# saifahmadgit/go2-sim2real-locomotion-rl

Hardware: AMD Instinct MI355X
Metric: env-steps/sec (all envs) Go2 walk 4096 envs; 1/2/4/8-GPU scaling (higher is better)
Workload: dtype f32

## Files before the change

### go2_sim2real_locomotion_rl_amd/build.py

```python
import os
import shutil
import subprocess
import sys

_HERE = os.path.dirname(os.path.abspath(__file__))
REPO_ROOT = os.path.dirname(_HERE)
HIP_SRC = os.path.join(_HERE, "csrc", "go2sim.hip")
HIP_SRC_POLICY = os.path.join(_HERE, "csrc", "go2sim_policy.hip")
HIP_HDR_GJK = os.path.join(_HERE, "csrc", "go2sim_gjk_dev.h")
HIP_LIB = os.path.join(_HERE, "csrc", "libgo2sim.so")
ORACLE_SRC = os.path.join(REPO_ROOT, "oracle", "go2sim_cpu.cpp")
ORACLE_SRC_POLICY = os.path.join(REPO_ROOT, "oracle", "policy_cpu.cpp")
ORACLE_LIB = os.path.join(REPO_ROOT, "oracle", "libgo2sim_cpu.so")
ORACLE_LIB_FAST = os.path.join(REPO_ROOT, "oracle", "libgo2sim_cpu_fast.so")

HIP_FLAGS = ["--offload-arch=gfx950", "-O3", "-std=c++17", "-ffp-contract=off", "-fPIC", "-shared", "-Wall", "-Wno-unused-function",
             "-Wno-unused-const-variable"]
CPU_FLAGS = ["-O2", "-std=c++17", "-ffp-contract=off", "-fopenmp", "-fPIC", "-shared", "-Wall", "-Wno-unused-function", "-Wno-unused-variable"]


def _newer(target, *sources):
    if not os.path.exists(target):
        return False
    t = os.path.getmtime(target)
# ... 36 lines not shown
        cmd = ["g++", *CPU_FLAGS, *extra, ORACLE_SRC, ORACLE_SRC_POLICY, "-o", lib]
        if verbose:
            print("[build]", " ".join(cmd), file=sys.stderr)
        subprocess.run(cmd, check=True)
    return ORACLE_LIB


def build_oracle_variant(name, extra_flags, force=False, verbose=True):
    out = os.path.join(REPO_ROOT, "oracle", f"libgo2sim_cpu_{name}.so")
    deps = [ORACLE_SRC, ORACLE_SRC_POLICY, os.path.join(REPO_ROOT, "oracle", "gjk_epa_cpu.h"), *_headers()]
    if not force and _newer(out, *deps):
        return out
    cmd = ["g++", *CPU_FLAGS, *extra_flags, ORACLE_SRC, ORACLE_SRC_POLICY, "-o", out]
    if verbose:
        print("[build]", " ".join(cmd), file=sys.stderr)
    subprocess.run(cmd, check=True)
    return out


HIP_VARIANTS = {
    "bracket_inline": ["-DGO2SIM_BRACKET_INLINE"],
    "rng_const": ["-DGO2SIM_RNG_CONST"],
    "strict": ["-DGO2SIM_FAST_ORDER=0"],
}
ORACLE_VARIANTS = {
    "rng_const": ["-DGO2SIM_RNG_CONST"],
    "rng_const_fast": ["-DGO2SIM_RNG_CONST", "-DGO2SIM_FAST_ORDER"],
}


SHAPES = {
    "pendulum": dict(NL=3, ND=1, NQ=1, NG=2, NJ=1),
    "double_pendulum": dict(NL=4, ND=2, NQ=2, NG=3, NJ=2),
    "box": dict(NL=2, ND=6, NQ=7, NG=2, NJ=1),
}


def _shape_flags(name):
    return [f"-DGO2SIM_{k}={v}" for k, v in SHAPES[name].items()]


def build_shape_variant(name, hip=True, force=False, verbose=True):
    cpu = build_oracle_variant("shape_" + name, _shape_flags(name), force=force, verbose=verbose)
    gpu = build_hip_variant("shape_" + name, ["-DGO2SIM_FAST_ORDER=0", *_shape_flags(name)], force=force, verbose=verbose) if hip else None
    return cpu, gpu

# ... 22 lines not shown
```

### go2_sim2real_locomotion_rl_amd/csrc/go2sim.hip

```cpp

#include <hip/hip_runtime.h>

#include <cstdint>
#include <cstdio>
#include <cstdlib>
#include <cstring>
#include <new>
#include <vector>

#include "../../include/go2sim.h"
#include "../../include/go2sim_detmath.h"

#define DEV __device__ __forceinline__
#define DEVN __device__ __noinline__

namespace {

constexpr int NL = GO2SIM_NL, ND = GO2SIM_ND, NQ = GO2SIM_NQ, NG = GO2SIM_NG, NJ = GO2SIM_NJ;
constexpr int NPAIR = GO2SIM_NPAIR_MAX, MAXC = GO2SIM_MAX_CONTACTS, MAXB = GO2SIM_MAX_BROAD, MAXR = GO2SIM_MAX_ROWS;
constexpr int JOINT_FIXED = 0, JOINT_REVOLUTE = 1, JOINT_FREE = 4;
constexpr int GEOM_PLANE = 0, GEOM_SPHERE = 1, GEOM_CYLINDER = 3, GEOM_BOX = 5, GEOM_TERRAIN = 7;
constexpr int TERRAIN_CB = 4;
constexpr int MAX_CONTACTS_PER_PAIR = 5;
constexpr int CTRL_FORCE = 0, CTRL_VELOCITY = 1, CTRL_POSITION = 2;
// ... 168 lines not shown
  ovel = cross(s_ang, m_vel) + cross(s_vel, m_ang);
  oang = cross(s_ang, m_ang);
}
DEV void orthogonals(V3 a, V3& b, V3& c) {
  if (dm_abs(a.y) < 0.5f) b = v3(-a.x * a.y, 1.0f - a.y * a.y, -a.z * a.y);
  else b = v3(-a.x * a.z, -a.y * a.z, 1.0f - a.z * a.z);
  b = normalized(b);
  c = cross(a, b);
}
DEV void imp_aref(const float* p, float neg_penetration, float vel, float pos, float& imp, float& aref) {
  float timeconst = p[0], dampratio = p[1], dmin = p[2], dmax = p[3], width = p[4], mid = p[5], power = p[6];
  float imp_x = dm_abs(neg_penetration) / width;
  float imp_a = (1.0f / dm_pow(mid, power - 1.0f)) * dm_pow(imp_x, power);
  float imp_b = 1.0f - (1.0f / dm_pow(1.0f - mid, power - 1.0f)) * dm_pow(1.0f - imp_x, power);
  float imp_y = (imp_x < mid) ? imp_a : imp_b;
  imp = dmin + imp_y * (dmax - dmin);
  imp = clampf(imp, dmin, dmax);
  imp = (imp_x > 1.0f) ? dmax : imp;
  float b = 2.0f / (dmax * timeconst);
  float k = 1.0f / (dmax * dmax * timeconst * timeconst * dampratio * dampratio);
  aref = -b * vel - k * imp * pos;
}

struct Link {
  int parent, root, entity, is_fixed, joint_start, joint_end, dof_start, dof_end, q_start, q_end, n_dofs, geom_start, geom_end;
  V3 pos; Q4 quat; V3 inertial_pos; Q4 inertial_quat; M3 inertial_i; float mass; float invweight[2];
};
struct Joint { int type, link, q_start, dof_start, dof_end; V3 pos; float sol_params[7]; };
struct Dof { V3 motion_ang, motion_vel; float limit[2], invweight, armature, damping, stiffness, frictionloss, kp, kv, force_range[2]; };
struct Geom { int type, link, is_convex; V3 pos; Q4 quat; float data[7], friction, sol_params[7]; V3 center; V3 aabb[8]; float rim[32][2]; };
struct Entity { int link_start, link_end, dof_start, dof_end, geom_start, geom_end; };
struct Model {
  int n_links, n_joints, n_dofs, n_qs, n_geoms, n_entities, n_pairs, max_collision_pairs, max_contact_pairs, max_broad_pairs,
      n_contacts_per_pair, iterations, ls_iterations, ccd_iterations, support_res;
  float substep_dt; V3 gravity; float eps, tolerance, ls_tolerance, meaninertia, mc_perturbation, mc_tolerance, mpr_to_gjk_ratio, ccd_eps,
      ccd_tolerance;
  Link links[NL]; Joint joints[NJ]; Dof dofs[ND]; Geom geoms[NG]; Entity entities[2];
  float qpos0[NQ]; float mass_parent_mask[ND][ND]; int pair_idx[NG][NG]; int theta_to_ring[180];
  int pair_list[NPAIR];
  int terrain_enabled, terrain_rows, terrain_cols; float terrain_hs; float terrain_xyz_maxmin[6]; const float* terrain_hf;
  const float* terrain_cmax; int terrain_crows, terrain_ccols;
  int n_levels, level_start[NL + 1], level_links[NL], child_start[NL + 1], child_list[NL], dof_link[ND];
  int arrow_mode;
};

bool parse_model(const void* blob, size_t nbytes, Model& m) {
  m.terrain_enabled = 0; m.terrain_rows = m.terrain_cols = 0; m.terrain_hs = 0.0f; m.terrain_hf = nullptr;
  m.terrain_cmax = nullptr; m.terrain_crows = m.terrain_ccols = 0;
  if (nbytes < 128) return false;
  const int32_t* H = (const int32_t*)blob;
  if (H[0] != GO2SIM_MODEL_MAGIC || H[1] != GO2SIM_MODEL_VERSION) return false;
  m.n_links = H[2]; m.n_joints = H[3]; m.n_dofs = H[4]; m.n_qs = H[5]; m.n_geoms = H[6]; m.n_entities = H[7];
  m.n_pairs = H[8]; m.max_collision_pairs = H[9]; m.max_contact_pairs = H[10]; m.max_broad_pairs = H[11];
  m.n_contacts_per_pair = H[12]; m.iterations = H[13]; m.ls_iterations = H[14]; m.ccd_iterations = H[15]; m.support_res = H[16];
  int nf = H[18], ni = H[19];
  if (m.n_links != NL || m.n_joints != NJ || m.n_dofs != ND || m.n_qs != NQ || m.n_geoms != NG || m.n_entities != 2) return false;
  if (m.n_pairs > NPAIR || m.max_contact_pairs > MAXC || m.max_broad_pairs > MAXB || m.support_res != 180 || H[17] != 32) return false;
  if (m.n_contacts_per_pair > MAX_CONTACTS_PER_PAIR) return false;
  if (nbytes < 128 + (size_t)4 * (nf + ni)) return false;
  const float* F = (const float*)((const char*)blob + 128);
  const int32_t* I = (const int32_t*)(F + nf);
  const float* f = F;
  m.substep_dt = f[0]; m.gravity = {f[1], f[2], f[3]}; m.eps = f[4]; m.tolerance = f[5]; m.ls_tolerance = f[6]; m.meaninertia = f[7];
  m.mc_perturbation = f[8]; m.mc_tolerance = f[9]; m.mpr_to_gjk_ratio = f[10]; m.ccd_eps = f[11]; m.ccd_tolerance = f[12];
  f += 16;
  for (int i = 0; i < NL; ++i, f += 26) {
// ... 61 lines not shown
    for (int i = 0; i < NL; ++i) {
      int par = m.links[i].parent;
      if (par >= i) return false;
      depth[i] = (par < 0) ? 0 : depth[par] + 1;
      if (depth[i] > max_depth) max_depth = depth[i];
    }
    m.n_levels = max_depth + 1;
    int k = 0;
    for (int lev = 0; lev <= max_depth; ++lev) {
      m.level_start[lev] = k;
      for (int i = 0; i < NL; ++i) if (depth[i] == lev) m.level_links[k++] = i;
    }
    for (int lev = max_depth + 1; lev <= NL; ++lev) m.level_start[lev] = k;
    k = 0;
    for (int par = 0; par < NL; ++par) {
      m.child_start[par] = k;
      for (int i = NL - 1; i > par; --i) if (m.links[i].parent == par) m.child_list[k++] = i;
    }
    m.child_start[NL] = k;
    for (int d = 0; d < ND; ++d) m.dof_link[d] = -1;
    for (int i = 0; i < NL; ++i) for (int d = m.links[i].dof_start; d < m.links[i].dof_end; ++d) m.dof_link[d] = i;
    for (int d = 0; d < ND; ++d) if (m.dof_link[d] < 0) return false;
  }
  int g_next = 0;
  for (int i = 0; i < NL; ++i) { if (m.links[i].geom_start != g_next) return false; g_next = m.links[i].geom_end; }
  return g_next == NG;
}


struct LinkS {
  int parent, entity, is_fixed, joint_start, joint_end, dof_start, dof_end, q_start, q_end, n_dofs;
  V3 pos; Q4 quat; V3 inertial_pos; Q4 inertial_quat; M3 inertial_i; float mass; float invweight[2];
};
struct GeomS { int type, link; V3 pos; Q4 quat; };
struct JLim { int q_start, dof_start; float lo, hi; };
constexpr int NTRI = ND * (ND + 1) / 2;
constexpr int LEG_K = 4, LEG_D = 3;
struct alignas(16) ModelS {
  int n_levels, iterations, ls_iterations, arrow_mode;
  float substep_dt; V3 gravity; float eps, tolerance, ls_tolerance, meaninertia;
  LinkS links[NL];
  unsigned char tri_i[NTRI + 1], tri_j[NTRI + 1];
  JLim jlim[NJ];
  Joint joints[NJ]; Dof dofs[ND]; GeomS geoms[NG]; Entity entities[2];
  float qpos0[NQ]; unsigned mass_mask_bits[ND];
  int level_start[NL + 1], level_links[NL], child_start[NL + 1], child_list[NL], dof_link[ND];
// ... 62 lines not shown
      float v = m.mass_parent_mask[i][j];
      if (v == 1.0f) bits |= 1u << j; else if (v != 0.0f) return false;
    }
    o.mass_mask_bits[i] = bits;
  }
  for (int i = 0; i <= NL; ++i) { o.level_start[i] = m.level_start[i]; o.child_start[i] = m.child_start[i]; }
  for (int i = 0; i < NL; ++i) { o.level_links[i] = m.level_links[i]; o.child_list[i] = m.child_list[i]; }
  for (int i = 0; i < ND; ++i) o.dof_link[i] = m.dof_link[i];
  int k = 0;
  for (int i = 0; i < ND; ++i) for (int j = 0; j <= i; ++j) { o.tri_i[k] = (unsigned char)i; o.tri_j[k] = (unsigned char)j; k++; }
  for (int i = 0; i < NJ; ++i) {
    const Joint& J = m.joints[i];
    bool rev = J.type == JOINT_REVOLUTE;
    o.jlim[i].q_start = rev ? J.q_start : -1; o.jlim[i].dof_start = J.dof_start;
    o.jlim[i].lo = rev ? m.dofs[J.dof_start].limit[0] : 0.0f; o.jlim[i].hi = rev ? m.dofs[J.dof_start].limit[1] : 0.0f;
  }
  o.leg_form = build_leg_form(m, o) ? 1 : 0;
  return true;
}
DEV float mass_mask(const ModelS& m, int i, int j) { return (float)((m.mass_mask_bits[i] >> j) & 1u); }
DEV void tri_index(const ModelS& m, int idx, int& i, int& j) { i = m.tri_i[idx]; j = m.tri_j[idx]; }

struct ModelView {
  int n_levels, iterations, ls_iterations, arrow_mode, leg_form; float substep_dt; V3 gravity; float eps, tolerance, ls_tolerance, meaninertia;
  const LinkS* links; const Joint* joints; const Dof* dofs; const GeomS* geoms; const Entity* entities; const float* qpos0;
  const unsigned* mass_mask_bits; const int *level_start, *level_links, *child_start, *child_list, *dof_link; const unsigned char *tri_i, *tri_j;
  const unsigned char* leg_links; int leg_root;
  DEV ModelView(const ModelS* t, const ModelS* __restrict__ g)
      : n_levels(g->n_levels), iterations(g->iterations), ls_iterations(g->ls_iterations), arrow_mode(g->arrow_mode), leg_form(g->leg_form), substep_dt(g->substep_dt), gravity(g->gravity), eps(g->eps),
        tolerance(g->tolerance), ls_tolerance(g->ls_tolerance), meaninertia(g->meaninertia), links(t->links), joints(t->joints), dofs(t->dofs),
        geoms(t->geoms), entities(t->entities), qpos0(t->qpos0), mass_mask_bits(t->mass_mask_bits), level_start(t->level_start),
        level_links(t->level_links), child_start(t->child_start), child_list(t->child_list), dof_link(t->dof_link), tri_i(t->tri_i), tri_j(t->tri_j),
        leg_links(t->leg_links), leg_root(g->leg_root) {}
  DEV ModelView(const LinkS* lds_links, const unsigned char* lds_tri_i, const unsigned char* lds_tri_j, const Model* __restrict__ g)
      : n_levels(g->n_levels), iterations(g->iterations), ls_iterations(g->ls_iterations), arrow_mode(g->arrow_mode), leg_form(0), substep_dt(g->substep_dt), gravity(g->gravity), eps(g->eps),
        tolerance(g->tolerance), ls_tolerance(g->ls_tolerance), meaninertia(g->meaninertia), links(lds_links), joints(g->joints), dofs(g->dofs),
        geoms(nullptr), entities(g->entities), qpos0(g->qpos0), mass_mask_bits(nullptr), level_start(nullptr), level_links(nullptr), child_start(nullptr),
        child_list(nullptr), dof_link(nullptr), tri_i(lds_tri_i), tri_j(lds_tri_j), leg_links(nullptr), leg_root(-1) {}
};
DEV float mass_mask(const ModelView& m, int i, int j) { return (float)((m.mass_mask_bits[i] >> j) & 1u); }
DEV void tri_index(const ModelView& m, int idx, int& i, int& j) { i = m.tri_i[idx]; j = m.tri_j[idx]; }
constexpr int lds_dma_bytes(int nbytes) { return (nbytes + 1023) / 1024 * 1024; }
template <int NBYTES>
DEV void wg_dma_to_lds(void* lds_dst, const void* __restrict__ src, int lane = (int)threadIdx.x) {
#pragma unroll
  for (int k = 0; k < lds_dma_bytes(NBYTES) / 1024; ++k)
    __builtin_amdgcn_global_load_lds((const __attribute__((address_space(1))) void*)((const char*)src + (k * 64 + lane) * 16),
                                     (__attribute__((address_space(3))) void*)((char*)lds_dst + k * 1024), 16, 0, 0);
}
constexpr int MODELS_LDS_BYTES = lds_dma_bytes((int)sizeof(ModelS));

#define GO2SIM_FLOAT_FIELDS(X)                                                                                       \
  X(qpos, NQ) X(vel, ND) X(ctrl_force, ND) X(ext, NL * 6) X(mass_shift, NL) X(com_shift, NL * 3)                        \
  X(friction_ratio, NG) X(l_pos, NL * 3) X(l_quat, NL * 4) X(cd_vel, NL * 3) X(cd_ang, NL * 3) X(root_com, NL * 3)     \
  X(contact_force, NL * 3) X(geom_friction, NG) X(ctrl_pos, ND) X(ctrl_vel, ND) X(dof_pos, ND) \
                                                                                       \
  X(actions, NA) X(last_actions, NA) X(applied_actions, NA) X(action_history, GO2SIM_ACTION_RING_MAX * NA) X(target_dof_pos, NM)            \
  X(e_dof_pos, NM) X(e_dof_vel, NM) X(last_dof_vel, NM) X(torque, NM) X(base_pos, 3) X(base_quat, 4) X(base_lin_vel, 3) \
// ... 151 lines not shown
    team_stage_r<N, STRIDE, R + 1>(k0, ld, st);
    st(k, v);
  }
}
template <int N, int T, class FL, class FS>
DEV void team_stage(int tl, FL ld, FS st) { team_stage_r<N, T, 0>(tl, ld, st); }
template <int EPW, int COUNT, class F>
DEV void wg_load(const Pool& P, int b0, int off, F put) {
  const int ev = threadIdx.x % EPW, k0 = threadIdx.x / EPW;
  const int b = (b0 + ev < P.B) ? b0 + ev : P.B - 1;
  auto ld = [&](int k) { return P.f[(size_t)(off + k) * P.B + b]; };
  auto st = [&](int k, float v) { put(ev, k, v); };
  team_stage_r<COUNT, 64 / EPW, 0>(k0, ld, st);
}

#ifdef GO2SIM_PHASE_PROFILE
constexpr int PH_MAX_WG = 8192;
__device__ unsigned long long g_phase_cycles[PH_MAX_WG * 64];
#define PH_BEGIN unsigned long long ph_t = __builtin_readcyclecounter();
#define PH(i) { __builtin_amdgcn_s_waitcnt(0); unsigned long long ph_n = __builtin_readcyclecounter(); if (threadIdx.x == 0 && blockIdx.x < PH_MAX_WG) g_phase_cycles[blockIdx.x * 64 + (i)] += ph_n - ph_t; ph_t = __builtin_readcyclecounter(); }
#define PHD_BEGIN unsigned long long phd_t = __builtin_readcyclecounter();
#define PHD(i) { unsigned long long phd_n = __builtin_readcyclecounter(); const unsigned long long phd_a = __ballot(1); if ((int)threadIdx.x == __ffsll((long long)phd_a) - 1 && blockIdx.x < PH_MAX_WG) { atomicAdd(&g_phase_cycles[blockIdx.x * 64 + (i)], phd_n - phd_t); atomicAdd(&g_phase_cycles[blockIdx.x * 64 + (i) + 1], 1ull); } phd_t = __builtin_readcyclecounter(); }
#define PHC(i, n) { if (threadIdx.x == 0 && blockIdx.x < PH_MAX_WG) g_phase_cycles[blockIdx.x * 64 + (i)] += (unsigned long long)(n); }
#else
#define PH_BEGIN
#define PH(i)
#define PHD_BEGIN
#define PHD(i)
#define PHC(i, n)
#endif

#ifdef GO2SIM_STAMP
constexpr int ST_KINDS = 8, ST_MAX_WG = 4096, ST_DEPTH = 4;
__device__ unsigned long long g_stamp[ST_KINDS * ST_MAX_WG * ST_DEPTH * 2];
__device__ unsigned g_stamp_cnt[ST_KINDS * ST_MAX_WG];
struct StampScope {
  int kind; unsigned long long t0;
  DEV StampScope(int k) : kind(k) { t0 = __builtin_amdgcn_s_memrealtime(); }
  DEV ~StampScope() {
    __builtin_amdgcn_s_waitcnt(0);
    const unsigned long long t1 = __builtin_amdgcn_s_memrealtime();
    if (threadIdx.x == 0 && blockIdx.x < ST_MAX_WG) {
      const int w = kind * ST_MAX_WG + (int)blockIdx.x;
      const unsigned c = g_stamp_cnt[w];
      g_stamp[(w * ST_DEPTH + (int)(c % ST_DEPTH)) * 2] = t0; g_stamp[(w * ST_DEPTH + (int)(c % ST_DEPTH)) * 2 + 1] = t1;
      g_stamp_cnt[w] = c + 1;
    }
// ... 47 lines not shown
  for (int c = 0; c < LPT_CLS; ++c) {
    const int k = rec[x * LPT_CLS + c];
    if (cls < 0 && local < total + k) { cls = c; off = local - total; }
    total += k;
  }
  if (total != expected) return ident;
  if (cls < 0 || off >= cap) return B;
  return rec[8 * LPT_CLS + (x * LPT_CLS + cls) * cap + off] * epw + slot;
}

struct KinData {
  float qpos[NQ], vel[ND], qpos_next[NQ], vel_next[ND];
  float l_pos[NL * 3], l_quat[NL * 4], i_pos[NL * 3], i_quat[NL * 4];
  float xanchor[NJ * 3], xaxis[NJ * 3];
  float cdof_ang[ND * 3], cdof_vel[ND * 3];
  float cd_vel[NL * 3], cd_ang[NL * 3];
  float mass[NL];
  int valid;
};

#ifndef GO2SIM_FAST_ORDER
#define GO2SIM_FAST_ORDER 1
#endif
template <int CTRL>
DEV float dpp_perm(float x) { return __int_as_float(__builtin_amdgcn_update_dpp(0, __float_as_int(x), CTRL, 0xf, 0xf, true)); }
#if GO2SIM_FAST_ORDER
constexpr bool ARROW_SHAPE = (ND == 18);
DEV float leg_sum4(float x) {
  const auto r = __builtin_amdgcn_permlane16_swap(__float_as_uint(x), __float_as_uint(x), false, false);
  const float p = __uint_as_float(r[0]) + __uint_as_float(r[1]);
  return p + dpp_perm<0x128>(p);
}
DEV float4 lds4(const float* p) { return *(const float4*)p; }
template <int T, int STRIDE>
DEV void arrow_factor(const int mode, const float eps, const float* A, float* F, int tl) {
  static_assert(T == 32 || T == 64, "four groups of eight lanes");
  const int leg = (tl >> 3) & 3, u = tl & 7, ub = u < 6 ? u : 5;
  const int p0 = dm_arrow_dof(mode, leg, 0), p1 = dm_arrow_dof(mode, leg, 1), p2 = dm_arrow_dof(mode, leg, 2);
  const bool w_lane = tl < 32 && u < 6;
  const float a00 = A[p0 * STRIDE + p0], a10 = A[p1 * STRIDE + p0], a11 = A[p1 * STRIDE + p1];
  const float a20 = A[p2 * STRIDE + p0], a21 = A[p2 * STRIDE + p1], a22 = A[p2 * STRIDE + p2];
  const float c0 = A[p0 * STRIDE + ub], c1 = A[p1 * STRIDE + ub], c2 = A[p2 * STRIDE + ub];
  float br[6];
#pragma unroll
  for (int j = 0; j < 6; ++j) br[j] = A[ub * STRIDE + j];
  team_sync();
// ... 2207 lines not shown
      mask &= mask - 1ull;
      const float D = s->efc_D[c], sg = (s->active[c] != 0) ? 1.0f : -1.0f;
      float jd[3], jj[3];
#pragma unroll
      for (int a = 0; a < 3; ++a) { const float j1 = Ji[c * DS + a]; jd[a] = (dm_abs(j1) > m.eps) ? sg * (j1 * D) : 0.0f; jj[a] = Jj[c * DS + a]; }
#pragma unroll
      for (int a = 0; a < 3; ++a)
#pragma unroll
        for (int q = 0; q < 3; ++q) h[a][q] = __builtin_fmaf(jj[q], jd[a], h[a][q]);
    }
  }
  if (on) {
#pragma unroll
    for (int a = 0; a < 3; ++a)
#pragma unroll
      for (int q = 0; q < 3; ++q) {
        const int i = 3 * bi + a, j = 3 * bj + q;
        s->Ablk[blk * 9 + 3 * a + q] = h[a][q];
        if (j <= i) s->H[i * DS + j] = h[a][q];
      }
  }
  team_sync();
}
#else
template <int T, class S, class MT>
DEV void ts_hessian_direct(const MT& m, S* s, int tl, int n_con) {
  for (int idx = tl; idx < ND * (ND + 1) / 2; idx += T) {
    int i, j;
    tri_index(m, idx, i, j);
    float h = 0.0f;
#pragma unroll 16
    for (int c = 0; c < n_con; ++c) {
      float j1 = s->J[c * DS + i];
      float t = s->J[c * DS + j] * j1 * s->DA[c];
      h = (dm_abs(j1) > m.eps) ? (h + t) : h;
    }
    h = h + s->M[i * DS + j];
    s->H[i * DS + j] = h;
  }
  team_sync();
}
#endif

template <int T, class S, class MT>
DEV void ts_cholesky_factor_columns(const MT& m, S* s, int tl) {
#pragma unroll
// ... 646 lines not shown
        const float active = (float)(rw.Ja < 0.0f);
        const float xs[3] = {rw.q0 * active, rw.q1 * active, rw.q2 * active}, bs[3] = {t0, t1, t2};
        float tot[3];
        team_serial_sum<T, 3>(xs, bs, tl, nseg, tot);
        t0 = tot[0]; t1 = tot[1]; t2 = tot[2];
        done = true;
      }
    }
    if (!done) {
#pragma unroll 16
      for (int c = 0; c < n_con; ++c) {
        float active = (float)(s->Jaref[c] < 0.0f);
        t0 = t0 + s->qf0[c] * active; t1 = t1 + s->qf1[c] * active; t2 = t2 + s->qf2[c] * active;
      }
    }
    p0.alpha = 0.0f; p0.cost = t0; p0.grad = t1; p0.hess = 2.0f * t2;
    if (p0.hess <= 0.0f) p0.hess = m.eps;
  }
  LS_MARK(50)
  return ts_linesearch_tail<T>(m, s, tl, n_con, nseg, rw, gtol, qg0, qg1, qg2, p0);
}

#undef LS_MARK
template <int T, class S, class MT>
DEV int ts_solve(const MT& m, const E& e, S* s, int tl, int nc, int n_con, unsigned lim_mask, int ws_flag) {
  PH_BEGIN
  const bool ws = (n_con > 0) && ws_flag;
  team_stage<NTRI, T>(tl, [&](int k) { return aload(e, AO(mass_mat), k); }, [&](int k, float v) { int i, j; tri_index(m, k, i, j); s->M[i * DS + j] = v; s->M[j * DS + i] = v; });
  team_stage<ND * 3, T>(tl, [&](int k) { return aload(e, AO(cdof_ang), k); }, [&](int k, float v) { s->cdof_ang[k] = v; });
  team_stage<ND * 3, T>(tl, [&](int k) { return aload(e, AO(cdof_vel), k); }, [&](int k, float v) { s->cdof_vel[k] = v; });
  team_stage<NL * 3, T>(tl, [&](int k) { return gload(e, FO(root_com), k); }, [&](int k, float v) { s->root_com[k] = v; });
  team_stage<ND, T>(tl, [&](int d) { return gload(e, FO(vel), d); }, [&](int d, float v) { s->vel[d] = v; });
  team_stage<ND, T>(tl, [&](int d) { return aload(e, AO(force), d); }, [&](int d, float v) { s->force[d] = v; });
  team_stage<ND, T>(tl, [&](int d) { return aload(e, AO(acc_smooth), d); }, [&](int d, float v) { s->acc_smooth[d] = v; });
  team_stage<ND, T>(tl, [&](int d) { return aload(e, AO(qacc_ws), d); }, [&](int d, float v) { s->qacc[d] = v; });
  team_sync();
  if (!ws) team_for<ND, T>(tl, [&](int d) { s->qacc[d] = s->acc_smooth[d]; });
  team_sync();
  PH(0)
  bool rows_coupled = false;
  for (int r = tl; r < 4 * nc; r += T) {
    int i_col = r >> 2, i = r & 3;
    int link_a = e.c_link()[i_col], link_b = e.c_link()[MAXC + i_col];
    V3 cpos = e.c_pos()[i_col], cnormal = e.c_normal()[i_col];
    float friction = e.c_friction()[i_col], pen = e.c_pen()[i_col];
    float sol[7];
    auto csol = e.c_sol()[i_col];
#pragma unroll
    for (int k = 0; k < 7; ++k) sol[k] = csol[k];
    V3 d1, d2;
    orthogonals(cnormal, d1, d2);
    float invweight = m.links[link_a].invweight[0];
    if (link_b > -1) invweight = invweight + m.links[link_b].invweight[0];
    V3 d = (float)(2 * (i % 2) - 1) * ((i < 2) ? d1 : d2);
    V3 n = d * friction - cnormal;
    float* row = &s->J[r * DS];
#pragma unroll
    for (int i_d = 0; i_d < DS; ++i_d) row[i_d] = 0.0f;
    float jac_qvel = 0.0f;
    unsigned legs = 0u;
    for (int i_ab = 0; i_ab < 2; ++i_ab) {
      float sign = -1.0f; int link = link_a;
      if (i_ab == 1) { sign = 1.0f; link = link_b; }
      while (link > -1) {
        V3 t_pos = cpos - v3(s->root_com[3 * link], s->root_com[3 * link + 1], s->root_com[3 * link + 2]);
        const int nd = m.links[link].n_dofs, de = m.links[link].dof_end;
        if (nd > 0 && de > 6) legs |= 1u << dm_arrow_leg(m.arrow_mode, de - 1);
        for (int i_d_ = 0; i_d_ < nd; ++i_d_) {
          int i_d = de - 1 - i_d_;
          V3 ca = v3(s->cdof_ang[3 * i_d], s->cdof_ang[3 * i_d + 1], s->cdof_ang[3 * i_d + 2]);
          V3 cv = v3(s->cdof_vel[3 * i_d], s->cdof_vel[3 * i_d + 1], s->cdof_vel[3 * i_d + 2]);
          V3 velv = cv - cross(t_pos, ca);
          V3 diff = sign * velv;
          float j = dot(diff, n);
          jac_qvel = jac_qvel + j * s->vel[i_d];
          row[i_d] = row[i_d] + j;
        }
        link = m.links[link].parent;
      }
    }
    float imp, aref;
    imp_aref(sol, -pen, jac_qvel, -pen, imp, aref);
    float diag = invweight + friction * friction * invweight;
    diag *= 2.0f * friction * friction * (1.0f - imp) / imp;
    diag = fmx(diag, m.eps);
    s->aref[r] = aref; s->efc_D[r] = 1.0f / diag;
    rows_coupled = rows_coupled || (legs & (legs - 1u)) != 0u;
  }
  for (int i_j = tl; i_j < NJ; i_j += T) {
    if (!((lim_mask >> i_j) & 1u)) continue;
    const Joint& Jt = m.joints[i_j];
    int i_d = Jt.dof_start;
    float q = gload(e, FO(qpos), Jt.q_start);
    float pos_delta_min = q - m.dofs[i_d].limit[0];
    float pos_delta_max = m.dofs[i_d].limit[1] - q;
    float pos_delta = fmn(pos_delta_min, pos_delta_max);
    {
      int r = 4 * nc + __popc(lim_mask & ((1u << i_j) - 1u));
      float j = (float)((pos_delta_min < pos_delta_max) * 2 - 1);
      float jac_qvel = j * s->vel[i_d];
      float imp, aref;
      imp_aref(Jt.sol_params, pos_delta, jac_qvel, pos_delta, imp, aref);
      float diag = fmx(m.dofs[i_d].invweight * (1.0f - imp) / imp, m.eps);
      s->aref[r] = aref; s->efc_D[r] = 1.0f / diag;
      float* row = &s->J[r * DS];
#pragma unroll
      for (int i_d2 = 0; i_d2 < DS; ++i_d2) row[i_d2] = 0.0f;
      row[i_d] = j;
    }
  }
  team_sync();
  PH(1)
  {
    float qa[ND];
#pragma unroll
    for (int d = 0; d < ND; ++d) qa[d] = s->qacc[d];
    for (int d1 = tl; d1 < ND; d1 += T) {
      float Ma_ = 0.0f;
#pragma unroll
      for (int d2 = 0; d2 < ND; ++d2) Ma_ = Ma_ + s->M[d1 * DS + d2] * qa[d2];
      s->Ma[d1] = Ma_;
    }
    for (int c = tl; c < n_con; c += T) {
      float Jv = -s->aref[c];
#pragma unroll
      for (int d = 0; d < ND; ++d) Jv = Jv + s->J[c * DS + d] * qa[d];
      s->Jaref[c] = Jv;
    }
  }
  team_sync();
  float cost = 0.0f, prev_cost = 0.0f, gauss = 0.0f;
  ts_update_constraint<T>(m, s, tl, n_con, cost, prev_cost, gauss);
  PH(2)
  int iters = 0;
  if (n_con > 0) {
    const float tol_scaled = (m.meaninertia * (float)imx(1, ND)) * m.tolerance;
    bool need_full = true;
    [[maybe_unused]] bool arrow = false;
#if GO2SIM_FAST_ORDER
    if constexpr (ARROW_SHAPE && (T == 32 || T == 64)) arrow = m.arrow_mode != 0 && team_ballot<T>(rows_coupled) == 0ull;
#endif
    for (int it = 0;; ++it) {
      if (need_full) {
#if GO2SIM_FAST_ORDER
        if constexpr (T >= 21) { if (it == 0) ts_hessian_direct<T>(m, s, tl, n_con); else ts_hessian_update<T>(m, s, tl, n_con); }
        else ts_hessian_direct<T>(m, s, tl, n_con);
        PH(3)
        if constexpr (ARROW_SHAPE && (T == 32 || T == 64)) { if (arrow) ts_cholesky_factor_arrow<T>(m, s, tl); else ts_cholesky_factor<T>(m, s, tl); }
        else ts_cholesky_factor<T>(m, s, tl);
#else
        ts_hessian_direct<T>(m, s, tl, n_con);
        PH(3)
        ts_cholesky_factor<T>(m, s, tl);
#endif
        PH(4)
      }
#if GO2SIM_FAST_ORDER
      [[maybe_unused]] float grad_sq_arrow = 0.0f;
      if constexpr (ARROW_SHAPE && (T == 32 || T == 64)) { if (arrow) grad_sq_arrow = ts_update_gradient_arrow<T>(m, s, tl); else ts_update_gradient<T>(s, tl); }
      else ts_update_gradient<T>(s, tl);
#else
      ts_update_gradient<T>(s, tl);
#endif
      PH(5)
      if (it > 0) {
        float improvement = prev_cost - cost;
        float grad_norm = 0.0f;
        if constexpr (T >= 32) {
          const float g = s->grad[tl < ND ? tl : ND - 1];
// ... 74 lines not shown
    ((int*)cf)[4 * i_c + 3] = pre ? lk0 : (e.c_link()[i_c] | (e.c_link()[MAXC + i_c] << 8));
  }
  team_sync();
  for (int i_l = tl; i_l < NL; i_l += T) {
    V3 acc = v3(0, 0, 0);
#pragma unroll 4
    for (int i_c = 0; i_c < nc; ++i_c) {
      int lk = ((const int*)cf)[4 * i_c + 3];
      int la = lk & 0xff, lb = lk >> 8;
      V3 f = v3(cf[4 * i_c], cf[4 * i_c + 1], cf[4 * i_c + 2]);
      if (la == i_l) acc = acc - f;
      if (lb == i_l) acc = acc + f;
    }
    e.contact_force()[i_l] = acc;
  }
}

template <int T>
DEVN void ts_solve_overflow(float* Pf, int* Pi, int PB, float* Pfa, int* Pia, int b, const LinkS* lnk, const unsigned char* tri_i, const unsigned char* tri_j,
                            const Model* __restrict__ gm, SolverData<MAXR>* s, int tl, int nc, int n_con, unsigned lim_mask, int ws_flag) {
  Pool P; P.f = Pf; P.i = Pi; P.B = PB; P.fa = Pfa; P.ia = Pia;
  const E e(P, b);
  const ModelView m(lnk, tri_i, tri_j, gm);
  int iters = ts_solve<T>(m, e, s, tl, nc, n_con, lim_mask, ws_flag);
  ts_commit<T>(m, e, s, tl, nc, n_con, iters);
}

template <int T, int RLN>
DEV void solve_body(const Pool& P, const Model* __restrict__ gm, const ModelS* __restrict__ mp, SolverData<MAXR>* __restrict__ overflow,
                    const int* __restrict__ lpt_rec, int* __restrict__ lpt_next, int lpt_cap, SolverData<RLN>* lds, char* blk_raw, int& b_out, bool& resident_out) {
  constexpr int EPW = 64 / T;
  const LinkS* lnk = (const LinkS*)blk_raw;
  const unsigned char* tri_i = (const unsigned char*)(blk_raw + sizeof(LinkS) * NL);
  const unsigned char* tri_j = tri_i + (NTRI + 1);
  static_assert(T >= NJ, "one lane per joint in the limit test");
  PH_BEGIN
  wg_dma_to_lds<SOLVER_BLOCK_BYTES>(blk_raw, mp->links);
  const int tl = threadIdx.x % T, slot = threadIdx.x / T;
  const int b = lpt_take(lpt_rec, lpt_cap, P.B, EPW, slot);
  if (lpt_next && blockIdx.x == 0) for (int i = threadIdx.x; i < 8 * LPT_CLS; i += 64) lpt_next[i] = 0;
  const bool env_valid = b < P.B;
  b_out = b; resident_out = false;
  E e(P, env_valid ? b : P.B - 1);
  const int nc = e.n_contacts()[0];
  const int ws_flag = e.is_warmstart()[0];
  const JLim jl = mp->jlim[tl < NJ ? tl : NJ - 1];
  const float q_lim = gload(e, FO(qpos), jl.q_start < 0 ? 0 : jl.q_start);
  const bool lim = tl < NJ && jl.q_start >= 0 && fmn(q_lim - jl.lo, jl.hi - q_lim) < 0;
  const unsigned lim_mask = (unsigned)((__ballot(lim) >> (slot * T)) & ((T == 64) ? ~0ull : ((1ull << T) - 1ull)));
  const int n_lim = __popc(lim_mask);
  __syncthreads();
  PH(9)
  const ModelView m(lnk, tri_i, tri_j, gm);
  if (!env_valid) return;
  const int n_con = 4 * nc + n_lim;
  if (n_con <= RLN) {
    SolverData<RLN>* s = &lds[slot];
    resident_out = true;
    int iters = ts_solve<T>(m, e, s, tl, nc, n_con, lim_mask, ws_flag);
    PH(10)
    ts_commit<T>(m, e, s, tl, nc, n_con, iters);
    PH(11)
  } else {
    ts_solve_overflow<T>(P.f, P.i, P.B, P.fa, P.ia, b, lnk, tri_i, tri_j, gm, &overflow[b], tl, nc, n_con, lim_mask, ws_flag);
  }
}
template <int T, int RLN>
__global__ __launch_bounds__(64) __attribute__((amdgpu_waves_per_eu(2, 2))) void k_constraint_solve_team(Pool P, const Model* __restrict__ gm, const ModelS* __restrict__ mp, SolverData<MAXR>* __restrict__ overflow,
                                                                                                         const int* __restrict__ lpt_rec, int* __restrict__ lpt_next, int lpt_cap) {
  STAMP(STK_SOLVE)
  constexpr int EPW = 64 / T;
  __shared__ SolverData<RLN> lds[EPW];
  __shared__ alignas(16) char blk_raw[lds_dma_bytes(SOLVER_BLOCK_BYTES)];
  int b; bool resident;
  solve_body<T, RLN>(P, gm, mp, overflow, lpt_rec, lpt_next, lpt_cap, lds, blk_raw, b, resident);
}

constexpr size_t cmax(size_t a, size_t b) { return a > b ? a : b; }
template <int T, int RLN, bool WITH_DYN>
__global__ __launch_bounds__(64) __attribute__((amdgpu_waves_per_eu(2, 2))) void k_solve_integrate_team(Pool P, const Model* __restrict__ gm, const ModelS* __restrict__ mp,
                                                                                                        SolverData<MAXR>* __restrict__ overflow, const int* __restrict__ lpt_rec,
                                                                                                        int* __restrict__ lpt_next, int lpt_cap) {
  STAMP(STK_SOLVE)
  constexpr int EPW = 64 / T;
  constexpr size_t SOLVE_OFF = (sizeof(SolverData<RLN>) * EPW + 15) / 16 * 16, DYN_OFF = (sizeof(DynData) * EPW + 15) / 16 * 16, KIN_OFF = (sizeof(KinData) * EPW + 15) / 16 * 16;
  constexpr size_t SOLVE_BYTES = SOLVE_OFF + lds_dma_bytes(SOLVER_BLOCK_BYTES);
  constexpr size_t KSEP_OFF = (sizeof(KinSeparate<KIN_OVERLAY, EPW>) + 15) / 16 * 16;
  constexpr size_t DYN_BYTES = DYN_OFF + MODELS_LDS_BYTES + (BROAD_OVERLAY<T> ? sizeof(KinSeparate<KIN_OVERLAY, EPW>) : KSEP_OFF + sizeof(BroadSeparate<false, T>));
  constexpr size_t KIN_BYTES = KIN_OFF + MODELS_LDS_BYTES;
  __shared__ alignas(16) char raw[cmax(SOLVE_BYTES, WITH_DYN ? DYN_BYTES : KIN_BYTES)];
  const int tl = threadIdx.x % T, slot = threadIdx.x / T;
  int b; bool resident;
  SolverData<RLN>* lds = (SolverData<RLN>*)raw;
  solve_body<T, RLN>(P, gm, mp, overflow, lpt_rec, lpt_next, lpt_cap, lds, raw + SOLVE_OFF, b, resident);
  const bool pre = b < P.B && resident;
  const int dd = tl < ND ? tl : ND - 1;
  const float pre_vel = pre ? lds[slot].vel[dd] : 0.0f, pre_acc = pre ? lds[slot].qacc[dd] : 0.0f;
  __builtin_amdgcn_fence(__ATOMIC_RELEASE, "workgroup");
  __syncthreads();
  __builtin_amdgcn_fence(__ATOMIC_ACQUIRE, "workgroup");
  if constexpr (WITH_DYN) {
    DynData* lds_d = (DynData*)raw;
    char* ms_raw = raw + DYN_OFF;
    auto& lds_k = *(KinSeparate<KIN_OVERLAY, EPW>*)(ms_raw + MODELS_LDS_BYTES);
    auto& lds_b = *(BroadSeparate<BROAD_OVERLAY<T>, T>*)(ms_raw + MODELS_LDS_BYTES + KSEP_OFF);
    integrate_fk_dynamics_body<T>(P, mp, gm, b, lds_d, ms_raw, lds_k, lds_b, pre, pre_vel, pre_acc);
  } else {
    integrate_fk_body<T>(P, mp, b, (KinData*)raw, raw + KIN_OFF, pre, pre_vel, pre_acc);
  }
}

__global__ __launch_bounds__(64) void k_debug_narrowphase(const Model* __restrict__ mp, int which, int i_ga, int i_gb, V3 pa, Q4 qa, V3 pb, Q4 qb,
                                                          GjkStoreFull* __restrict__ full, float* __restrict__ out8) {
  __shared__ GjkStoreLds slots[GJK_SLOTS_MAX];
  __shared__ GjkStoreTeam team_store;
  __shared__ unsigned mask;
  if (threadIdx.x == 0) mask = 0u;
// ... 2349 lines not shown
```

Baseline: 17.71 million.

## Add sparse support-path Jacobian setup and group-masked Hessian for contact solver

```diff
diff --git a/go2_sim2real_locomotion_rl_amd/build.py b/go2_sim2real_locomotion_rl_amd/build.py
--- a/go2_sim2real_locomotion_rl_amd/build.py
+++ b/go2_sim2real_locomotion_rl_amd/build.py
@@ -82,6 +82,7 @@
     "bracket_inline": ["-DGO2SIM_BRACKET_INLINE"],
     "rng_const": ["-DGO2SIM_RNG_CONST"],
     "strict": ["-DGO2SIM_FAST_ORDER=0"],
+    "prof": ["-DGO2SIM_PHASE_PROFILE"],
 }
 ORACLE_VARIANTS = {
     "rng_const": ["-DGO2SIM_RNG_CONST"],
diff --git a/go2_sim2real_locomotion_rl_amd/csrc/go2sim.hip b/go2_sim2real_locomotion_rl_amd/csrc/go2sim.hip
--- a/go2_sim2real_locomotion_rl_amd/csrc/go2sim.hip
+++ b/go2_sim2real_locomotion_rl_amd/csrc/go2sim.hip
@@ -214,6 +214,7 @@
   aref = -b * vel - k * imp * pos;
 }
 
+constexpr int SUP_PATH = 9;
 struct Link {
   int parent, root, entity, is_fixed, joint_start, joint_end, dof_start, dof_end, q_start, q_end, n_dofs, geom_start, geom_end;
   V3 pos; Q4 quat; V3 inertial_pos; Q4 inertial_quat; M3 inertial_i; float mass; float invweight[2];
@@ -234,6 +235,7 @@
   const float* terrain_cmax; int terrain_crows, terrain_ccols;
   int n_levels, level_start[NL + 1], level_links[NL], child_start[NL + 1], child_list[NL], dof_link[ND];
   int arrow_mode;
+  int support_setup;
 };
 
 bool parse_model(const void* blob, size_t nbytes, Model& m) {
@@ -341,6 +343,12 @@
     for (int i = 0; i < NL; ++i) for (int d = m.links[i].dof_start; d < m.links[i].dof_end; ++d) m.dof_link[d] = i;
     for (int d = 0; d < ND; ++d) if (m.dof_link[d] < 0) return false;
   }
+  m.support_setup = (m.arrow_mode != 0 && !(getenv("GO2SIM_NO_SUPPORT_SETUP") && atoi(getenv("GO2SIM_NO_SUPPORT_SETUP")) != 0)) ? 1 : 0;
+  for (int i = 0; i < NL; ++i) {
+    int n_path = 0;
+    for (int l = i; l > -1; l = m.links[l].parent) n_path += m.links[l].n_dofs;
+    if (n_path > SUP_PATH) m.support_setup = 0;
+  }
   int g_next = 0;
   for (int i = 0; i < NL; ++i) { if (m.links[i].geom_start != g_next) return false; g_next = m.links[i].geom_end; }
   return g_next == NG;
@@ -449,18 +457,18 @@
 DEV void tri_index(const ModelS& m, int idx, int& i, int& j) { i = m.tri_i[idx]; j = m.tri_j[idx]; }
 
 struct ModelView {
-  int n_levels, iterations, ls_iterations, arrow_mode, leg_form; float substep_dt; V3 gravity; float eps, tolerance, ls_tolerance, meaninertia;
+  int n_levels, iterations, ls_iterations, arrow_mode, leg_form, support_setup; float substep_dt; V3 gravity; float eps, tolerance, ls_tolerance, meaninertia;
   const LinkS* links; const Joint* joints; const Dof* dofs; const GeomS* geoms; const Entity* entities; const float* qpos0;
   const unsigned* mass_mask_bits; const int *level_start, *level_links, *child_start, *child_list, *dof_link; const unsigned char *tri_i, *tri_j;
   const unsigned char* leg_links; int leg_root;
   DEV ModelView(const ModelS* t, const ModelS* __restrict__ g)
-      : n_levels(g->n_levels), iterations(g->iterations), ls_iterations(g->ls_iterations), arrow_mode(g->arrow_mode), leg_form(g->leg_form), substep_dt(g->substep_dt), gravity(g->gravity), eps(g->eps),
+      : n_levels(g->n_levels), iterations(g->iterations), ls_iterations(g->ls_iterations), arrow_mode(g->arrow_mode), leg_form(g->leg_form), support_setup(0), substep_dt(g->substep_dt), gravity(g->gravity), eps(g->eps),
         tolerance(g->tolerance), ls_tolerance(g->ls_tolerance), meaninertia(g->meaninertia), links(t->links), joints(t->joints), dofs(t->dofs),
         geoms(t->geoms), entities(t->entities), qpos0(t->qpos0), mass_mask_bits(t->mass_mask_bits), level_start(t->level_start),
         level_links(t->level_links), child_start(t->child_start), child_list(t->child_list), dof_link(t->dof_link), tri_i(t->tri_i), tri_j(t->tri_j),
         leg_links(t->leg_links), leg_root(g->leg_root) {}
   DEV ModelView(const LinkS* lds_links, const unsigned char* lds_tri_i, const unsigned char* lds_tri_j, const Model* __restrict__ g)
-      : n_levels(g->n_levels), iterations(g->iterations), ls_iterations(g->ls_iterations), arrow_mode(g->arrow_mode), leg_form(0), substep_dt(g->substep_dt), gravity(g->gravity), eps(g->eps),
+      : n_levels(g->n_levels), iterations(g->iterations), ls_iterations(g->ls_iterations), arrow_mode(g->arrow_mode), leg_form(0), support_setup(g->support_setup), substep_dt(g->substep_dt), gravity(g->gravity), eps(g->eps),
         tolerance(g->tolerance), ls_tolerance(g->ls_tolerance), meaninertia(g->meaninertia), links(lds_links), joints(g->joints), dofs(g->dofs),
         geoms(nullptr), entities(g->entities), qpos0(g->qpos0), mass_mask_bits(nullptr), level_start(nullptr), level_links(nullptr), child_start(nullptr),
         child_list(nullptr), dof_link(nullptr), tri_i(lds_tri_i), tri_j(lds_tri_j), leg_links(nullptr), leg_root(-1) {}
@@ -658,7 +666,9 @@
 #define PHD_BEGIN unsigned long long phd_t = __builtin_readcyclecounter();
 #define PHD(i) { unsigned long long phd_n = __builtin_readcyclecounter(); const unsigned long long phd_a = __ballot(1); if ((int)threadIdx.x == __ffsll((long long)phd_a) - 1 && blockIdx.x < PH_MAX_WG) { atomicAdd(&g_phase_cycles[blockIdx.x * 64 + (i)], phd_n - phd_t); atomicAdd(&g_phase_cycles[blockIdx.x * 64 + (i) + 1], 1ull); } phd_t = __builtin_readcyclecounter(); }
 #define PHC(i, n) { if (threadIdx.x == 0 && blockIdx.x < PH_MAX_WG) g_phase_cycles[blockIdx.x * 64 + (i)] += (unsigned long long)(n); }
+#define PH_RESET { ph_t = __builtin_readcyclecounter(); }
 #else
+#define PH_RESET
 #define PH_BEGIN
 #define PH(i)
 #define PHD_BEGIN
@@ -752,6 +762,8 @@
 #ifndef GO2SIM_FAST_ORDER
 #define GO2SIM_FAST_ORDER 1
 #endif
+constexpr int SUP_FLAG = 10;
+constexpr bool SUPPORT_SETUP = GO2SIM_FAST_ORDER && ND == 18;
 template <int CTRL>
 DEV float dpp_perm(float x) { return __int_as_float(__builtin_amdgcn_update_dpp(0, __float_as_int(x), CTRL, 0xf, 0xf, true)); }
 #if GO2SIM_FAST_ORDER
@@ -3005,6 +3017,80 @@
   }
   team_sync();
 }
+template <int T, class S, class MT>
+DEV void ts_hessian_support(const MT& m, S* s, int tl) {
+  constexpr int NB = 21, G = (T >= 3 * NB) ? 3 : 1, NA = (G == 3) ? 3 : 1, NU = 3 * NB, NR = (G == 3) ? 2 : 4;
+  const unsigned long long* gm = (const unsigned long long*)s->jv;
+  static_assert(T == 32 || T == 64, "teams of 32 or 64 lanes");
+  using RM = typename std::conditional<T == 64, unsigned long long, unsigned>::type;
+  for (int u0 = 0; u0 < NU; u0 += T) {
+    const int u = u0 + tl;
+    const bool on = u < NU;
+    const int uu = on ? u : 0;
+    const int g = (G == 3) ? uu / NB : 0, blk = (G == 3) ? uu - NB * g : uu / 3, a0 = (G == 3) ? 0 : uu - 3 * blk;
+    const int bi = (blk >= 15) ? 5 : (blk >= 10) ? 4 : (blk >= 6) ? 3 : (blk >= 3) ? 2 : (blk >= 1) ? 1 : 0;
+    const int bj = blk - bi * (bi + 1) / 2;
+    RM rows = 0;
+#pragma unroll
+    for (int a = 0; a < NA; ++a) {
+      const int i = 3 * bi + a0 + a, gi = (i < 6) ? 4 : dm_arrow_leg(m.arrow_mode, i);
+      rows |= (RM)gm[gi];
+    }
+    if constexpr (G == 3) rows &= (RM)(0x9249249249249249ull << g);
+    if (!on) rows = 0;
+    float h[NA][3];
+#pragma unroll
+    for (int a = 0; a < NA; ++a)
+#pragma unroll
+      for (int q = 0; q < 3; ++q) h[a][q] = 0.0f;
+    const float* Ji = &s->J[3 * bi + a0];
+    const float* Jj = &s->J[3 * bj];
+    while (rows != 0) {
+      int c[NR]; bool ok[NR];
+#pragma unroll
+      for (int k = 0; k < NR; ++k) {
+        ok[k] = rows != 0;
+        if constexpr (T == 64) c[k] = ok[k] ? __ffsll((long long)rows) - 1 : 0; else c[k] = ok[k] ? __ffs((int)rows) - 1 : 0;
+        rows &= rows - 1;
+      }
+      float D[NR], j1[NR][NA], jj[NR][3];
+#pragma unroll
+      for (int k = 0; k < NR; ++k) {
+        D[k] = s->DA[c[k]];
+#pragma unroll
+        for (int a = 0; a < NA; ++a) j1[k][a] = Ji[c[k] * DS + a];
+#pragma unroll
+        for (int q = 0; q < 3; ++q) jj[k][q] = Jj[c[k] * DS + q];
+      }
+#pragma unroll
+      for (int k = 0; k < NR; ++k)
+#pragma unroll
+        for (int a = 0; a < NA; ++a) {
+          const float jd = (dm_abs(j1[k][a]) > m.eps) ? j1[k][a] * D[k] : 0.0f;
+#pragma unroll
+          for (int q = 0; q < 3; ++q) { const float hn = __builtin_fmaf(jj[k][q], jd, h[a][q]); h[a][q] = ok[k] ? hn : h[a][q]; }
+        }
+    }
+    if constexpr (G == 3) {
+#pragma unroll
+      for (int a = 0; a < NA; ++a)
+#pragma unroll
+        for (int q = 0; q < 3; ++q) { const float p1 = __shfl(h[a][q], tl + NB, T), p2 = __shfl(h[a][q], tl + 2 * NB, T); h[a][q] = (h[a][q] + p1) + p2; }
+    }
+    if (on && g == 0) {
+#pragma unroll
+      for (int a = 0; a < NA; ++a)
+#pragma unroll
+        for (int q = 0; q < 3; ++q) {
+          const int i = 3 * bi + a0 + a, j = 3 * bj + q;
+          const float v = h[a][q] + s->M[i * DS + j];
+          s->Ablk[blk * 9 + 3 * (a0 + a) + q] = v;
+          if (j <= i) s->H[i * DS + j] = v;
+        }
+    }
+  }
+  team_sync();
+}
 #else
 template <int T, class S, class MT>
 DEV void ts_hessian_direct(const MT& m, S* s, int tl, int n_con) {
@@ -3697,7 +3783,7 @@
 }
 
 #undef LS_MARK
-template <int T, class S, class MT>
+template <int T, bool SUP = true, class S, class MT>
 DEV int ts_solve(const MT& m, const E& e, S* s, int tl, int nc, int n_con, unsigned lim_mask, int ws_flag) {
   PH_BEGIN
   const bool ws = (n_con > 0) && ws_flag;
@@ -3714,7 +3800,101 @@
   team_sync();
   PH(0)
   bool rows_coupled = false;
-  for (int r = tl; r < 4 * nc; r += T) {
+  [[maybe_unused]] bool sup_rows = false;
+  [[maybe_unused]] unsigned row_groups = 0u;
+  [[maybe_unused]] bool row_bad = false;
+  if constexpr (SUP && SUPPORT_SETUP && (T == 32 || T == 64)) {
+    if (m.support_setup != 0) {
+      bool two_sided = false;
+      for (int c = tl; c < nc; c += T) {
+        const int link_a = e.c_link()[c], link_b = e.c_link()[MAXC + c];
+        ((int*)s->qf0)[c] = link_a | (link_b << 8);
+        int n_side = 0;
+        for (int i_ab = 0; i_ab < 2; ++i_ab) {
+          bool has = false;
+          for (int link = i_ab ? link_b : link_a; link > -1; link = m.links[link].parent) has = has || m.links[link].n_dofs > 0;
+          n_side += has ? 1 : 0;
+        }
+        two_sided = two_sided || n_side == 2;
+      }
+      sup_rows = team_ballot<T>(two_sided) == 0ull;
+    }
+    if (sup_rows) {
+      for (int r = tl; r < 4 * nc; r += T) {
+        float4* row4 = (float4*)&s->J[r * DS];
+#pragma unroll
+        for (int k = 0; k < DS / 4; ++k) row4[k] = make_float4(0.0f, 0.0f, 0.0f, 0.0f);
+      }
+      team_sync();
+      for (int u = tl; u < SUP_PATH * nc; u += T) {
+        const int i_col = u / SUP_PATH;
+        int k = u - SUP_PATH * i_col;
+        const int link_ab = ((const int*)s->qf0)[i_col], link_a = link_ab & 0xff, link_b = link_ab >> 8;
+        const V3 cpos = e.c_pos()[i_col], cnormal = e.c_normal()[i_col];
+        const float friction = e.c_friction()[i_col];
+        int i_d = -1, link_d = 0; float sign = -1.0f;
+        for (int i_ab = 0; i_ab < 2; ++i_ab)
+          for (int link = i_ab ? link_b : link_a; link > -1 && i_d < 0; link = m.links[link].parent) {
+            const int nd = m.links[link].n_dofs;
+            if (k < nd) { i_d = m.links[link].dof_end - 1 - k; link_d = link; sign = i_ab ? 1.0f : -1.0f; }
+            k -= nd;
+          }
+        if (i_d < 0) continue;
+        V3 d1, d2;
+        orthogonals(cnormal, d1, d2);
+        V3 t_pos = cpos - v3(s->root_com[3 * link_d], s->root_com[3 * link_d + 1], s->root_com[3 * link_d + 2]);
+        V3 ca = v3(s->cdof_ang[3 * i_d], s->cdof_ang[3 * i_d + 1], s->cdof_ang[3 * i_d + 2]);
+        V3 cv = v3(s->cdof_vel[3 * i_d], s->cdof_vel[3 * i_d + 1], s->cdof_vel[3 * i_d + 2]);
+        V3 velv = cv - cross(t_pos, ca);
+        V3 diff = sign * velv;
+#pragma unroll
+        for (int i = 0; i < 4; ++i) {
+          V3 d = (float)(2 * (i % 2) - 1) * ((i < 2) ? d1 : d2);
+          V3 n = d * friction - cnormal;
+          float j = dot(diff, n);
+          s->J[(4 * i_col + i) * DS + i_d] = 0.0f + j;
+        }
+      }
+      team_sync();
+      for (int r = tl; r < 4 * nc; r += T) {
+        const int i_col = r >> 2;
+        const int link_ab = ((const int*)s->qf0)[i_col], link_a = link_ab & 0xff, link_b = link_ab >> 8;
+        const float friction = e.c_friction()[i_col], pen = e.c_pen()[i_col];
+        float sol[7];
+        auto csol = e.c_sol()[i_col];
+#pragma unroll
+        for (int k = 0; k < 7; ++k) sol[k] = csol[k];
+        float invweight = m.links[link_a].invweight[0];
+        if (link_b > -1) invweight = invweight + m.links[link_b].invweight[0];
+        const float* row = &s->J[r * DS];
+        float jac_qvel = 0.0f;
+        unsigned groups = 0u;
+        for (int i_ab = 0; i_ab < 2; ++i_ab)
+          for (int link = i_ab ? link_b : link_a; link > -1; link = m.links[link].parent) {
+            const int nd = m.links[link].n_dofs, de = m.links[link].dof_end;
+            if (nd > 0) groups |= (de > 6) ? 1u << dm_arrow_leg(m.arrow_mode, de - 1) : 16u;
+            for (int t0 = 0; t0 < nd; t0 += 6) {
+              float jr[6], vr[6];
+#pragma unroll
+              for (int t = 0; t < 6; ++t) { const int i_d = (t0 + t < nd) ? de - 1 - t0 - t : 0; jr[t] = row[i_d]; vr[t] = s->vel[i_d]; }
+#pragma unroll
+              for (int t = 0; t < 6; ++t) { const float sum = jac_qvel + jr[t] * vr[t]; jac_qvel = (t0 + t < nd) ? sum : jac_qvel; }
+            }
+          }
+        float imp, aref;
+        imp_aref(sol, -pen, jac_qvel, -pen, imp, aref);
+        float diag = invweight + friction * friction * invweight;
+        diag *= 2.0f * friction * friction * (1.0f - imp) / imp;
+        diag = fmx(diag, m.eps);
+        const float D = 1.0f / diag;
+        s->aref[r] = aref; s->efc_D[r] = D;
+        rows_coupled = rows_coupled || ((groups & 15u) & ((groups & 15u) - 1u)) != 0u;
+        row_groups = groups;
+        row_bad = row_bad || !(dm_abs(jac_qvel) < __builtin_inff()) || !(dm_abs(D) < __builtin_inff());
+      }
+    }
+  }
+  for (int r = tl; r < (sup_rows ? 0 : 4 * nc); r += T) {
     int i_col = r >> 2, i = r & 3;
     int link_a = e.c_link()[i_col], link_b = e.c_link()[MAXC + i_col];
     V3 cpos = e.c_pos()[i_col], cnormal = e.c_normal()[i_col];
@@ -3734,6 +3914,7 @@
     for (int i_d = 0; i_d < DS; ++i_d) row[i_d] = 0.0f;
     float jac_qvel = 0.0f;
     unsigned legs = 0u;
+    [[maybe_unused]] unsigned base = 0u;
     for (int i_ab = 0; i_ab < 2; ++i_ab) {
       float sign = -1.0f; int link = link_a;
       if (i_ab == 1) { sign = 1.0f; link = link_b; }
@@ -3741,6 +3922,7 @@
         V3 t_pos = cpos - v3(s->root_com[3 * link], s->root_com[3 * link + 1], s->root_com[3 * link + 2]);
         const int nd = m.links[link].n_dofs, de = m.links[link].dof_end;
         if (nd > 0 && de > 6) legs |= 1u << dm_arrow_leg(m.arrow_mode, de - 1);
+        if (nd > 0 && de <= 6) base = 16u;
         for (int i_d_ = 0; i_d_ < nd; ++i_d_) {
           int i_d = de - 1 - i_d_;
           V3 ca = v3(s->cdof_ang[3 * i_d], s->cdof_ang[3 * i_d + 1], s->cdof_ang[3 * i_d + 2]);
@@ -3761,6 +3943,8 @@
     diag = fmx(diag, m.eps);
     s->aref[r] = aref; s->efc_D[r] = 1.0f / diag;
     rows_coupled = rows_coupled || (legs & (legs - 1u)) != 0u;
+    row_groups = legs | base;
+    row_bad = row_bad || !(dm_abs(jac_qvel) < __builtin_inff()) || !(dm_abs(1.0f / diag) < __builtin_inff());
   }
   for (int i_j = tl; i_j < NJ; i_j += T) {
     if (!((lim_mask >> i_j) & 1u)) continue;
@@ -3784,6 +3968,27 @@
       row[i_d] = j;
     }
   }
+  if constexpr (SUP && SUPPORT_SETUP && (T == 32 || T == 64)) {
+    bool sup_hess = false;
+    if (m.support_setup != 0 && n_con <= T && n_con > 0) {
+      sup_hess = team_ballot<T>(row_bad) == 0ull;
+      unsigned long long gm[5];
+#pragma unroll
+      for (int g = 0; g < 5; ++g) gm[g] = team_ballot<T>(tl < 4 * nc && ((row_groups >> g) & 1u) != 0u);
+      int r = 4 * nc;
+      for (unsigned lm = lim_mask; lm != 0u; lm &= lm - 1u, ++r) {
+        const int i_d = m.joints[__ffs((int)lm) - 1].dof_start, gd = (i_d < 6) ? 4 : dm_arrow_leg(m.arrow_mode, i_d);
+#pragma unroll
+        for (int g = 0; g < 5; ++g) gm[g] |= (gd == g) ? 1ull << r : 0ull;
+      }
+      if (tl == 0) {
+#pragma unroll
+        for (int g = 0; g < 5; ++g) ((unsigned long long*)s->jv)[g] = gm[g];
+      }
+    }
+    if (tl == 0 && n_con > 0) ((int*)s->jv)[SUP_FLAG] = sup_hess ? 1 : 0;
+    if (n_con > 0) { PHC(10, sup_hess && sup_rows ? 1ull : 1ull << 32) }
+  }
   team_sync();
   PH(1)
   {
@@ -3818,8 +4023,11 @@
     for (int it = 0;; ++it) {
       if (need_full) {
 #if GO2SIM_FAST_ORDER
-        if constexpr (T >= 21) { if (it == 0) ts_hessian_direct<T>(m, s, tl, n_con); else ts_hessian_update<T>(m, s, tl, n_con); }
-        else ts_hessian_direct<T>(m, s, tl, n_con);
+        if constexpr (T >= 21) {
+          if (it > 0) ts_hessian_update<T>(m, s, tl, n_con);
+          else if constexpr (SUP && SUPPORT_SETUP && (T == 32 || T == 64)) { if (((const int*)s->jv)[SUP_FLAG] != 0) ts_hessian_support<T>(m, s, tl); else ts_hessian_direct<T>(m, s, tl, n_con); }
+          else ts_hessian_direct<T>(m, s, tl, n_con);
+        } else ts_hessian_direct<T>(m, s, tl, n_con);
         PH(3)
         if constexpr (ARROW_SHAPE && (T == 32 || T == 64)) { if (arrow) ts_cholesky_factor_arrow<T>(m, s, tl); else ts_cholesky_factor<T>(m, s, tl); }
         else ts_cholesky_factor<T>(m, s, tl);
@@ -3940,7 +4148,7 @@
   Pool P; P.f = Pf; P.i = Pi; P.B = PB; P.fa = Pfa; P.ia = Pia;
   const E e(P, b);
   const ModelView m(lnk, tri_i, tri_j, gm);
-  int iters = ts_solve<T>(m, e, s, tl, nc, n_con, lim_mask, ws_flag);
+  int iters = ts_solve<T, false>(m, e, s, tl, nc, n_con, lim_mask, ws_flag);
   ts_commit<T>(m, e, s, tl, nc, n_con, iters);
 }
 
@@ -3976,8 +4184,11 @@
     SolverData<RLN>* s = &lds[slot];
     resident_out = true;
     int iters = ts_solve<T>(m, e, s, tl, nc, n_con, lim_mask, ws_flag);
-    PH(10)
-    ts_commit<T>(m, e, s, tl, nc, n_con, iters);
+    PH_RESET
+    int b_commit = b;
+    asm volatile("" : "+v"(b_commit));
+    const E e_commit(P, b_commit);
+    ts_commit<T>(m, e_commit, s, tl, nc, n_con, iters);
     PH(11)
   } else {
     ts_solve_overflow<T>(P.f, P.i, P.B, P.fa, P.ia, b, lnk, tri_i, tri_j, gm, &overflow[b], tl, nc, n_con, lim_mask, ws_flag);
@@ -4011,6 +4222,7 @@
   int b; bool resident;
   SolverData<RLN>* lds = (SolverData<RLN>*)raw;
   solve_body<T, RLN>(P, gm, mp, overflow, lpt_rec, lpt_next, lpt_cap, lds, raw + SOLVE_OFF, b, resident);
+  asm volatile("" : "+v"(b));
   const bool pre = b < P.B && resident;
   const int dd = tl < ND ? tl : ND - 1;
   const float pre_vel = pre ? lds[slot].vel[dd] : 0.0f, pre_acc = pre ? lds[slot].qacc[dd] : 0.0f;
```

Result: slower. 17.26 million (-2.5%).
